# Siyou-Li/u2Tokenizer

Hardware: NVIDIA H100
Metric: ct_volumes_per_sec (higher is better)
Workload: dtype bf16

## Files before the change

include/u2b200.h:

```cpp
#ifndef U2B200_H_
#define U2B200_H_

#include <stdint.h>

#if defined(__GNUC__)
#define U2_API __attribute__((visibility("default")))
#else
#define U2_API
#endif

#ifdef __cplusplus
extern "C" {
#endif

#define U2_OK 0
#define U2_ERR_ARG (-1)
#define U2_ERR_CUDA (-2)
#define U2_ERR_UNSUPPORTED (-3)

#define U2_DT_BF16 0
#define U2_DT_F32 1

#define U2_ACT_NONE 0
#define U2_ACT_GELU 1
#define U2_ACT_SILU 2

#define U2_EPI_NONE 0
#define U2_EPI_EXP_ROW 1
#define U2_EPI_DS_ROW 2

U2_API int u2_version(void);
U2_API const char* u2_last_error(void);
U2_API int u2_device_sm_count(void);

typedef struct u2_gemm_desc {
  int32_t M, N, K;
  int32_t zi, zo;
  int32_t b_zi_div;
  int64_t lda, a_stride_zi, a_stride_zo;
  int64_t ldb, b_stride_zi, b_stride_zo;
  int64_t ldc, c_stride_zi, c_stride_zo;
  int32_t c_dtype;
  float alpha;
  const float* bias;
  int32_t act;
  const void* residual;
  int64_t ldr;
  int32_t res_row_mod;
  int32_t row_div, row_stride, row_off;
  int32_t block_n;
  int32_t a_mn, b_mn;
  int32_t epi_op;
  const float* rowvec;
  int64_t rv_stride_zi, rv_stride_zo;
  const void* mul;
} u2_gemm_desc;

U2_API int u2_gemm_bf16(const void* A, const void* B, void* C, const u2_gemm_desc* desc, void* stream);

U2_API int u2_layernorm_bf16(const void* x, const void* residual, const float* gamma, const float* beta,
                             void* y, void* sum_out, int64_t rows, int32_t E, int64_t ldx, int64_t ldr,
                             int64_t ldy, float eps, void* stream);
U2_API int u2_rmsnorm_bf16(const void* x, const void* residual, const float* gamma, void* y, void* sum_out,
                           int64_t rows, int32_t E, int64_t ldx, int64_t ldr, int64_t ldy, float eps,
                           void* stream);

// ... 271 lines not shown
```

u2tokenizer_b200/_lib.py:

```python
from __future__ import annotations

import ctypes as C
from pathlib import Path

_LIB_PATH = Path(__file__).resolve().parent / "libu2b200.so"
_lib = None


class GemmDesc(C.Structure):
    _fields_ = [
        ("M", C.c_int32), ("N", C.c_int32), ("K", C.c_int32),
        ("zi", C.c_int32), ("zo", C.c_int32), ("b_zi_div", C.c_int32),
        ("lda", C.c_int64), ("a_stride_zi", C.c_int64), ("a_stride_zo", C.c_int64),
        ("ldb", C.c_int64), ("b_stride_zi", C.c_int64), ("b_stride_zo", C.c_int64),
        ("ldc", C.c_int64), ("c_stride_zi", C.c_int64), ("c_stride_zo", C.c_int64),
        ("c_dtype", C.c_int32), ("alpha", C.c_float),
        ("bias", C.c_void_p),
        ("act", C.c_int32),
        ("residual", C.c_void_p),
        ("ldr", C.c_int64),
        ("res_row_mod", C.c_int32),
        ("row_div", C.c_int32), ("row_stride", C.c_int32), ("row_off", C.c_int32),
        ("block_n", C.c_int32),
        ("a_mn", C.c_int32), ("b_mn", C.c_int32),
# ... 176 lines not shown

BEAM_MAX_BEAMS, BEAM_MAX_EOS, BEAM_MAX_KEEP = 16, 8, 144


class BeamParams(C.Structure):
    _fields_ = [
        ("length_penalty", C.c_double),
        ("num_beams", C.c_int32), ("beams_to_keep", C.c_int32), ("early_stopping", C.c_int32),
        ("max_new_tokens", C.c_int32), ("n_eos", C.c_int32), ("reserved", C.c_int32),
        ("eos", C.c_int32 * BEAM_MAX_EOS),
    ]


class BeamStepDesc(C.Structure):
    _fields_ = [
        ("params", C.c_void_p),
        ("prompts", C.c_int32), ("V", C.c_int32),
        ("cand_val", C.c_void_p), ("cand_tok", C.c_void_p),
        ("running", C.c_void_p), ("fin_score", C.c_void_p), ("fin_info", C.c_void_p), ("flags", C.c_void_p),
        ("ids", C.c_void_p),
        ("rec", C.c_void_p), ("ld_rec", C.c_int64), ("rec_rows", C.c_int32),
        ("kv_src", C.c_void_p), ("ld_kv_src", C.c_int64),
        ("pos_dev", C.c_void_p),
        ("hist", C.c_void_p), ("ld_hist", C.c_int64), ("hist_cap", C.c_int32),
        ("step_dev", C.c_void_p),
    ]


_P, _I, _L, _F = C.c_void_p, C.c_int32, C.c_int64, C.c_float
SIGNATURES = {
    "u2_version": (C.c_int, []),
    "u2_last_error": (C.c_char_p, []),
    "u2_device_sm_count": (C.c_int, []),
    "u2_gemm_bf16": (C.c_int, [_P, _P, _P, C.POINTER(GemmDesc), _P]),
    "u2_layernorm_bf16": (C.c_int, [_P, _P, _P, _P, _P, _P, _L, _I, _L, _L, _L, _F, _P]),
    "u2_rmsnorm_bf16": (C.c_int, [_P, _P, _P, _P, _P, _L, _I, _L, _L, _L, _F, _P]),
    "u2_softmax_f32_bf16": (C.c_int, [_P, _P, C.POINTER(SoftmaxDesc), _P]),
    "u2_silu_mul_bf16": (C.c_int, [_P, _P, _L, _I, _L, _L, _I, _P]),
    "u2_patchify_f32_bf16": (C.c_int, [_P, _P, _L, _I, _I, _I, _I, _I, _I, _P]),
    "u2_patch_embed_f32_bf16": (C.c_int, [_P, _P, _P, _P, _P, _L, _I, _I, _I, _I, _I, _I, _I, _L, _P]),
    "u2_set_rows_bf16": (C.c_int, [_P, _P, _L, _L, _L, _I, _P]),
    "u2_vit_frame_rows_bf16": (C.c_int, [_P, _P, _L, _I, _I, _I, _P]),
    "u2_transpose_heads_bf16": (C.c_int, [_P, _P, _I, _I, _I, _I, _L, _L, _L, _L, _L, _L, _P]),
    "u2_spp_pool_bf16": (C.c_int, [_P, _P, _L, _I, _I, _I, _I, _I, _L, _L, _L, _I, _P]),
    "u2_multiscale_pool_bf16": (C.c_int, [_P, _P, _P, _F, _P, _I, _I, _I, _I, _P]),
    "u2_multiscale_pool_ws_elems": (C.c_int64, [_I, _I]),
    "u2_embed_splice_bf16": (C.c_int, [_P, _P, _P, _P, _I, _I, _I, _I, _L, _P]),
    "u2_temporal_attention_bf16": (C.c_int, [_P, _P, _I, _I, _I, _I, _I, _L, _L, _F, _P, _I, _P]),
    "u2_rope_bf16": (C.c_int, [_P, C.POINTER(RopeDesc), _P]),
    "u2_decode_attention_bf16": (C.c_int, [_P, _P, _P, _P, _I, _I, _I, _I, _I, _I, _P, _L, _L, _F, _I, _P, _L, _P]),
    "u2_decode_attention_window_bf16": (C.c_int, [_P, _P, _P, _P, _I, _I, _I, _I, _I, _I, _P, _L, _L, _F, _I, _P, _L,
                                                  _I, _P]),
    "u2_gemv_bf16": (C.c_int, [_P, _P, _P, C.POINTER(GemvDesc), _P]),
    "u2_argmax_f32": (C.c_int, [_P, _P, _P, _I, _I, _L, _P]),
    "u2_dlinear_bf16": (C.c_int, [_P, _P, _P, C.POINTER(DlinearDesc), _P]),
    "u2_decode_attention_fused_bf16": (C.c_int, [_P, _P, _P, _P, C.POINTER(FusedDecodeDesc), _P]),
    "u2_decode_embed_bf16": (C.c_int, [_P, _P, _P, _P, _P, _P, _P, _P, _I, _I, _L, _P]),
    "u2_flash_attention_d64_bf16": (C.c_int, [_P, _P, _P, _P, C.POINTER(FaDesc), _P]),
    "u2_sample_f32": (C.c_int, [_P, _P, _I, _I, _L, _F, _I, _F, C.c_uint64, _P, _I, _P]),
    "u2_sample_dev_f32": (C.c_int, [_P, _P, _I, _I, _L, _P, _P, _I, _P]),
    "u2_logits_process_f32": (C.c_int, [_P, _I, _I, _L, _P, _P, _L, _I, _P, _P, _I, _P]),
    "u2_topk_rows_f32": (C.c_int, [_P, _P, _I, _I, _I, _L, _L, _P]),
    "u2_log_softmax_f32": (C.c_int, [_P, _P, _I, _I, _L, _L, _P]),
    "u2_beam_topk_f32": (C.c_int, [_P, _L, _I, _I, _P, _P, _P, _P, _P, _P]),
    "u2_beam_step": (C.c_int, [C.POINTER(BeamStepDesc), _I, _P]),
    "u2_dlinear_ws_elems": (C.c_int64, [_I, _I]),
# ... 79 lines not shown
```

u2tokenizer_b200/csrc/attn_small.cu:

```cuda
#include <cooperative_groups.h>
#include <cuda_bf16.h>
#include <math.h>

#include <type_traits>

#include "host_util.h"
#include "u2b200.h"

namespace u2 {

__device__ __forceinline__ float wsum(float v) {
#pragma unroll
  for (int o = 16; o > 0; o >>= 1) v += __shfl_xor_sync(0xffffffffu, v, o);
  return v;
}
__device__ __forceinline__ float wmax(float v) {
#pragma unroll
  for (int o = 16; o > 0; o >>= 1) v = fmaxf(v, __shfl_xor_sync(0xffffffffu, v, o));
  return v;
}

__global__ void __launch_bounds__(128)
temporal_attention_kernel(const __nv_bfloat16* __restrict__ qkv, __nv_bfloat16* __restrict__ out, int C, int N,
                          int H, int dh, long long ld_qkv, long long ld_out, float scale,
// ... 545 lines not shown
      }
    }
  }
#pragma unroll
  for (int g = 0; g < kG; ++g) {
    if (lane == 0) {
      s_m[warp][g] = m[g];
      s_l[warp][g] = l[g];
    }
    if (kLanes == 32 || lane < kLanes) {
#pragma unroll
      for (int i = 0; i < kEpl; ++i) s_acc[warp][g][lane * kEpl + i] = acc[g][i];
    }
  }
  __syncthreads();
  for (int idx = threadIdx.x; idx < kG * kDh; idx += blockDim.x) {
    const int g = idx / kDh, e = idx - g * kDh;
    float gm = -INFINITY;
#pragma unroll
    for (int w = 0; w < kFaWarps; ++w) gm = fmaxf(gm, s_m[w][g]);
    float gl = 0.f, o = 0.f;
#pragma unroll
    for (int w = 0; w < kFaWarps; ++w) {
      if (s_m[w][g] != -INFINITY) {
        const float f = __expf(s_m[w][g] - gm);
        gl += s_l[w][g] * f;
        o += s_acc[w][g][e] * f;
      }
    }
    a.out[(long long)b * a.ldo + (long long)(hk * kG + g) * kDh + e] = __float2bfloat16(o / gl);
  }
}

template <int kDh, int kG, bool kInd, bool kWin = false>
__global__ void __launch_bounds__(256)
fused_decode_attention_split_kernel(const FusedArgsT<kInd, kWin> a) {
  namespace cg = cooperative_groups;
  cg::cluster_group cluster = cg::this_cluster();
  constexpr int kW = 8;
  constexpr int kEpl = PvMap<kDh>::kEpl;
  constexpr int kLanes = PvMap<kDh>::kLanes;
  constexpr int kVw = (kEpl + 1) / 2;
  const int S = (int)gridDim.z, rank = (int)blockIdx.z;
  const int hk = blockIdx.x, b = blockIdx.y;
  const int warp = threadIdx.x >> 5, lane = threadIdx.x & 31;
  const int le = kLanes == 32 ? lane : min(lane, kLanes - 1);
  asm volatile("griddepcontrol.launch_dependents;" ::: "memory");
  const int pos = a.pos_dev ? a.pos_dev[a.pos_per_seq ? b : 0] : a.pos_host;
  const int T = min(pos + 1, a.Tmax);
  const int lo = window_lo<kWin>(a, pos);
  __shared__ __align__(16) float s_q[kG][kDh];
  __shared__ __align__(16) __nv_bfloat16 s_knew[kDh];
  __shared__ __align__(16) __nv_bfloat16 s_vnew[kDh];
  __shared__ float s_m[kW][kG], s_l[kW][kG];
  __shared__ float s_acc[kW][kG][kDh];
  __shared__ float c_m[kG], c_l[kG];
  __shared__ __align__(16) float c_o[kG][kDh];

  const __nv_bfloat16* row = a.qkv + (long long)b * a.ldq;
  __nv_bfloat16* kbase = a.kc + ((long long)b * a.Hkv + hk) * a.Tmax * kDh;
  __nv_bfloat16* vbase = a.vc + ((long long)b * a.Hkv + hk) * a.Tmax * kDh;

  uint4 ku[kDh / 8];
  uint32_t vw[32][kVw];
  int t0 = (lo & ~31) + (warp * S + rank) * 32;
  const long long row_elems = (long long)a.Hkv * a.Tmax * kDh;
  auto request = [&](int base) {
    const int t = min(base + lane, T - 1);
    const long long dsrc = kv_src_delta<kInd>(a, b, t, pos, row_elems);
    const uint4* kr = reinterpret_cast<const uint4*>(kbase + (long long)t * kDh + dsrc);
#pragma unroll
    for (int c = 0; c < kDh / 8; ++c) ku[c] = kr[c];
#pragma unroll
    for (int jj = 0; jj < 32; ++jj) {
      const int tj = min(base + jj, T - 1);
      long long dj = 0;
      if constexpr (kInd) dj = __shfl_sync(0xffffffffu, dsrc, tj - base);
      const __nv_bfloat16* vp = vbase + (long long)tj * kDh + dj + le * kEpl;
      if constexpr (kEpl == 4) {
        const uint2 u = *reinterpret_cast<const uint2*>(vp);
        vw[jj][0] = u.x;
        vw[jj][1] = u.y;
      } else if constexpr (kEpl == 2) {
        vw[jj][0] = *reinterpret_cast<const uint32_t*>(vp);
      } else {
        vw[jj][0] = *reinterpret_cast<const unsigned short*>(vp);
      }
    }
  };
  if (t0 < T) request(t0);
  asm volatile("griddepcontrol.wait;" ::: "memory");

  for (int job = warp; job < kG + 2; job += kW) {
    if (job == kG) {
      norm_rope_head<kDh>(row + (long long)(a.Hq + hk) * kDh, a.k_norm_w, a.eps, a.inv_freq, pos, 1.f, nullptr, s_knew, lane);
      __syncwarp();
      if (rank == 0)
        for (int e = lane; e < kDh; e += 32) kbase[(long long)pos * kDh + e] = s_knew[e];
    } else if (job == kG + 1) {
      const __nv_bfloat16* v = row + (long long)(a.Hq + a.Hkv + hk) * kDh;
      for (int e = lane; e < kDh; e += 32) {
        const __nv_bfloat16 x = v[e];
        s_vnew[e] = x;
        if (rank == 0) vbase[(long long)pos * kDh + e] = x;
      }
    } else {
      norm_rope_head<kDh>(row + (long long)(hk * kG + job) * kDh, a.q_norm_w, a.eps, a.inv_freq, pos, a.scale, s_q[job],
                          nullptr, lane);
    }
  }
  __syncthreads();

  float m[kG], l[kG], acc[kG][kEpl];
#pragma unroll
  for (int g = 0; g < kG; ++g) {
    m[g] = -INFINITY;
    l[g] = 0.f;
#pragma unroll
    for (int i = 0; i < kEpl; ++i) acc[g][i] = 0.f;
  }
  while (t0 < T) {
    const int t = t0 + lane;
    if (t == pos) {
#pragma unroll
      for (int c = 0; c < kDh / 8; ++c) ku[c] = reinterpret_cast<const uint4*>(s_knew)[c];
    }
    float s[kG];
#pragma unroll
    for (int g = 0; g < kG; ++g) s[g] = 0.f;
#pragma unroll
    for (int c = 0; c < kDh / 8; ++c) {
      const __nv_bfloat162* h2 = reinterpret_cast<const __nv_bfloat162*>(&ku[c]);
      float kf[8];
#pragma unroll
      for (int j = 0; j < 4; ++j) {
        const float2 f2 = __bfloat1622float2(h2[j]);
        kf[2 * j] = f2.x;
        kf[2 * j + 1] = f2.y;
      }
#pragma unroll
      for (int g = 0; g < kG; ++g) {
        const float4 q0 = *reinterpret_cast<const float4*>(&s_q[g][c * 8]);
        const float4 q1 = *reinterpret_cast<const float4*>(&s_q[g][c * 8 + 4]);
        s[g] += kf[0] * q0.x + kf[1] * q0.y + kf[2] * q0.z + kf[3] * q0.w + kf[4] * q1.x + kf[5] * q1.y + kf[6] * q1.z +
                kf[7] * q1.w;
      }
    }
    float p[kG];
    const bool vis = t < T && (!kWin || t >= lo);
#pragma unroll
    for (int g = 0; g < kG; ++g) {
      if (!vis) s[g] = -INFINITY;
      const float mx = fmaxf(m[g], wmax(s[g]));
      const float corr = __expf(m[g] - mx);
      p[g] = vis ? __expf(s[g] - mx) : 0.f;
      l[g] = l[g] * corr + wsum(p[g]);
#pragma unroll
      for (int i = 0; i < kEpl; ++i) acc[g][i] *= corr;
      m[g] = mx;
    }
#pragma unroll
    for (int jj = 0; jj < 32; ++jj) {
      float vf[kEpl];
      if (t0 + jj == pos) {
#pragma unroll
        for (int i = 0; i < kEpl; ++i) vf[i] = __bfloat162float(s_vnew[le * kEpl + i]);
      } else if constexpr (kEpl == 4) {
        const float2 x = __bfloat1622float2(*reinterpret_cast<const __nv_bfloat162*>(&vw[jj][0]));
        const float2 y = __bfloat1622float2(*reinterpret_cast<const __nv_bfloat162*>(&vw[jj][1]));
        vf[0] = x.x; vf[1] = x.y; vf[2] = y.x; vf[3] = y.y;
      } else if constexpr (kEpl == 2) {
        const float2 x = __bfloat1622float2(*reinterpret_cast<const __nv_bfloat162*>(&vw[jj][0]));
        vf[0] = x.x; vf[1] = x.y;
      } else {
        vf[0] = __uint_as_float(vw[jj][0] << 16);
      }
#pragma unroll
      for (int g = 0; g < kG; ++g) {
        const float pj = __shfl_sync(0xffffffffu, p[g], jj);
#pragma unroll
        for (int i = 0; i < kEpl; ++i) acc[g][i] += pj * vf[i];
      }
    }
    t0 += S * kW * 32;
    if (t0 < T) request(t0);
  }
#pragma unroll
  for (int g = 0; g < kG; ++g) {
    if (lane == 0) {
      s_m[warp][g] = m[g];
      s_l[warp][g] = l[g];
    }
    if (kLanes == 32 || lane < kLanes) {
#pragma unroll
      for (int i = 0; i < kEpl; ++i) s_acc[warp][g][lane * kEpl + i] = acc[g][i];
    }
  }
  __syncthreads();
  for (int idx = threadIdx.x; idx < kG * kDh; idx += blockDim.x) {
    const int g = idx / kDh, e = idx - g * kDh;
    float gm = -INFINITY;
#pragma unroll
    for (int w = 0; w < kW; ++w) gm = fmaxf(gm, s_m[w][g]);
    float gl = 0.f, o = 0.f;
#pragma unroll
    for (int w = 0; w < kW; ++w) {
      if (s_m[w][g] != -INFINITY) {
        const float f = __expf(s_m[w][g] - gm);
        gl += s_l[w][g] * f;
        o += s_acc[w][g][e] * f;
      }
    }
    c_o[g][e] = o;
    if (e == 0) {
      c_m[g] = gm;
      c_l[g] = gl;
    }
  }
  cluster.sync();
  if (rank == 0) {
    for (int idx = threadIdx.x; idx < kG * kDh; idx += blockDim.x) {
      const int g = idx / kDh, e = idx - g * kDh;
      float gm = -INFINITY;
      for (int r = 0; r < S; ++r) gm = fmaxf(gm, *cluster.map_shared_rank(&c_m[g], r));
      float gl = 0.f, o = 0.f;
      for (int r = 0; r < S; ++r) {
        const float mr = *cluster.map_shared_rank(&c_m[g], r);
        if (mr != -INFINITY) {
          const float f = __expf(mr - gm);
          gl += *cluster.map_shared_rank(&c_l[g], r) * f;
          o += *cluster.map_shared_rank(&c_o[g][e], r) * f;
        }
      }
      a.out[(long long)b * a.ldo + (long long)(hk * kG + g) * kDh + e] = __float2bfloat16(o / gl);
    }
  }
  cluster.sync();
}

template <int kDh, int kG, bool kInd, bool kWin>
static int launch_fused_decode_split(const FusedArgsT<kInd, kWin>& a, dim3 grid, bool pdl, cudaStream_t st) {
  cudaLaunchConfig_t cfg = {};
  cfg.gridDim = grid;
  cfg.blockDim = dim3(256);
  cfg.dynamicSmemBytes = 0;
  cfg.stream = st;
  cudaLaunchAttribute attr[2];
  attr[0].id = cudaLaunchAttributeClusterDimension;
  attr[0].val.clusterDim.x = 1;
  attr[0].val.clusterDim.y = 1;
  attr[0].val.clusterDim.z = grid.z;
  attr[1].id = cudaLaunchAttributeProgrammaticStreamSerialization;
  attr[1].val.programmaticStreamSerializationAllowed = 1;
  cfg.attrs = attr;
  cfg.numAttrs = pdl ? 2 : 1;
  cudaError_t e = cudaLaunchKernelEx(&cfg, fused_decode_attention_split_kernel<kDh, kG, kInd, kWin>, a);
  if (e != cudaSuccess) return set_error(U2_ERR_CUDA, "decode_attention_fused (split-KV) launch: %s", cudaGetErrorString(e));
  return U2_OK;
}

template <int kDh, bool kInd, bool kWin = false>
static int launch_fused_decode(const FusedArgsT<kInd, kWin>& a, int G, dim3 grid, bool pdl, cudaStream_t st) {
  if (grid.z > 1) {
    switch (G) {
      case 1: return launch_fused_decode_split<kDh, 1, kInd, kWin>(a, grid, pdl, st);
      case 2: return launch_fused_decode_split<kDh, 2, kInd, kWin>(a, grid, pdl, st);
      case 4: return launch_fused_decode_split<kDh, 4, kInd, kWin>(a, grid, pdl, st);
      case 8: return launch_fused_decode_split<kDh, 8, kInd, kWin>(a, grid, pdl, st);
      default: return set_error(U2_ERR_UNSUPPORTED, "decode_attention_fused: Hq/Hkv = %d (supported 1, 2, 4, 8)", G);
    }
  }
  switch (G) {
    case 1: fused_decode_attention_kernel<kDh, 1, kInd, kWin><<<grid, FaCfg<kDh, 1>::kWarps * 32, 0, st>>>(a); break;
    case 2: fused_decode_attention_kernel<kDh, 2, kInd, kWin><<<grid, FaCfg<kDh, 2>::kWarps * 32, 0, st>>>(a); break;
    case 4: fused_decode_attention_kernel<kDh, 4, kInd, kWin><<<grid, FaCfg<kDh, 4>::kWarps * 32, 0, st>>>(a); break;
    case 8: fused_decode_attention_kernel<kDh, 8, kInd, kWin><<<grid, FaCfg<kDh, 8>::kWarps * 32, 0, st>>>(a); break;
    default: return set_error(U2_ERR_UNSUPPORTED, "decode_attention_fused: Hq/Hkv = %d (supported 1, 2, 4, 8)", G);
  }
  return U2_OK;
}

template <int kDh>
static int launch_fused_decode(const FusedDecodeWinArgs& a, int G, dim3 grid, bool pdl, cudaStream_t st) {
  if (a.window > 0) {
    if (a.kv_src) return launch_fused_decode<kDh, true, true>(a, G, grid, pdl, st);
    return launch_fused_decode<kDh, false, true>(a, G, grid, pdl, st);
  }
  if (a.kv_src) return launch_fused_decode<kDh, true>(static_cast<const FusedDecodeIndArgs&>(a), G, grid, pdl, st);
  return launch_fused_decode<kDh, false>(static_cast<const FusedDecodeArgs&>(a), G, grid, pdl, st);
// ... 42 lines not shown
```

u2tokenizer_b200/csrc/dlinear_wgmma.cu:

```cuda
#include <cuda_bf16.h>
#include <math.h>
#include <stdio.h>
#include <stdlib.h>

#include "host_util.h"
#include "ptx.cuh"
#include "u2b200.h"

namespace u2 {

constexpr int kDlN = 16;
constexpr int kDlK = 64;
constexpr int kDlBBytes = kDlN * kDlK * 2;
constexpr int kDlThreads = 384;
constexpr int kDlMmaWarp0 = 8;
constexpr int kDlAccLd = 20;

template <int kM>
struct DlCfg {
  static constexpr int kABytes = kM * kDlK * 2;
  static constexpr int kStageBytes = kABytes + kDlBBytes;
#ifndef U2_DL_STAGES128
#define U2_DL_STAGES128 10
#endif
  static constexpr int kStages = (kM == 128) ? U2_DL_STAGES128 : 18;
  static constexpr int kAccBytes = 2 * kM * kDlAccLd * 4;
  static constexpr int kSmem = kStages * kStageBytes + kAccBytes + 1024 + 512;
};

struct DlinArgs {
  int B, N, K;
  int num_tiles, kblocks;
  float* ws;
  int max_slots;
  int* counters;
  const float* ssq_in;
  float inv_norm_dim, eps;
  const __nv_bfloat16* residual;
  long long ldr;
  void* y;
  long long ldy;
  int y_dtype;
  int silu_pair;
  const float* gamma_next;
  __nv_bfloat16* xg;
  long long ldxg;
  float* ssq_out;
  float* ssq_part;
  int* ssq_ticket;
// ... 92 lines not shown
      it.kb = 0;
      it.left = 0;
    } else {
      const long long base = units * blockIdx.x / G;
      const long long end = units * (blockIdx.x + 1) / G;
      it.tile = (int)(base / kblocks);
      it.kb = (int)(base - (long long)it.tile * kblocks);
      it.left = (int)(end - base);
    }
  }
  return it;
}

__device__ __forceinline__ void wait_tile_flag(const int* flags, int t, int step, unsigned char* ready, int tag) {
  if (ready[t] == (unsigned char)tag) return;
  const int t4 = t & ~3;
  for (;;) {
    int4 f;
    asm volatile("ld.relaxed.gpu.global.v4.s32 {%0, %1, %2, %3}, [%4];"
                 : "=r"(f.x), "=r"(f.y), "=r"(f.z), "=r"(f.w)
                 : "l"(flags + t4)
                 : "memory");
    if (f.x >= step) ready[t4] = (unsigned char)tag;
    if (f.y >= step) ready[t4 + 1] = (unsigned char)tag;
    if (f.z >= step) ready[t4 + 2] = (unsigned char)tag;
    if (f.w >= step) ready[t4 + 3] = (unsigned char)tag;
    if (ready[t] == (unsigned char)tag) break;
  }
  asm volatile("fence.acq_rel.gpu;" ::: "memory");
  asm volatile("fence.proxy.async;" ::: "memory");
}

template <int kM>
__global__ void __launch_bounds__(kDlThreads, 1)
dlinear_wgmma_kernel(const __grid_constant__ DlinMulti mp) {
  using Cfg = DlCfg<kM>;
  constexpr int kStages = Cfg::kStages;
  constexpr int kABytes = Cfg::kABytes;
  constexpr int kStageBytes = Cfg::kStageBytes;
  constexpr bool kTiles = (kM == 64);
  extern __shared__ uint8_t smem_raw[];
  uint8_t* smem = reinterpret_cast<uint8_t*>((reinterpret_cast<uintptr_t>(smem_raw) + 1023) & ~static_cast<uintptr_t>(1023));
  uint8_t* smem_a = smem;
  uint8_t* smem_b = smem + kStages * kABytes;
  float* smem_acc = reinterpret_cast<float*>(smem + kStages * kStageBytes);
  uint64_t* bars = reinterpret_cast<uint64_t*>(smem + kStages * kStageBytes + Cfg::kAccBytes);
  uint64_t* full_bar = bars;
  uint64_t* empty_bar = bars + kStages;
  uint64_t* acc_full_bar = bars + 2 * kStages;
  uint64_t* acc_empty_bar = bars + 2 * kStages + 2;
  __shared__ unsigned char s_ready[1024];
  if (threadIdx.x < 256) reinterpret_cast<unsigned int*>(s_ready)[threadIdx.x] = 0u;

  const int warp_idx = threadIdx.x / 32;
  const int lane = threadIdx.x % 32;
  const int n_ops = mp.n_ops;

  if (warp_idx == 0 && lane == 0) {
    for (int i = 0; i < n_ops; ++i) {
      tma_prefetch_desc(&mp.tw[i]);
      tma_prefetch_desc(&mp.tx[i]);
    }
  }
  if (warp_idx == 1 && lane == 0) {
    for (int s = 0; s < kStages; ++s) {
      mbar_init(&full_bar[s], 1);
      mbar_init(&empty_bar[s], 4);
// ... 145 lines not shown
    uint32_t acc_phase = 0;
    for (int oi = 0; oi < n_ops; ++oi) {
      const DlinArgs& p = mp.op[oi];
      UnitIter it = make_iter(p.num_tiles, p.kblocks, kTiles);
      bool prev_done = (oi == 0);
      if (oi > 0 && !p.dep_flags) {
        if (et == 0) grid_barrier_wait(mp.gridbar + (oi - 1), target);
        asm volatile("bar.sync 1, 128;" ::: "memory");
        prev_done = true;
      }
      while (it.left > 0) {
        const int tile = it.tile;
        const int seg_kb = it.seg_len();
        it.left -= seg_kb;
        it.kb += seg_kb;
        if (it.kb == it.kblocks) {
          it.kb = 0;
          it.tile += it.tile_step;
        }

        const int row = tile * kM + trow;
        const bool whole = (seg_kb == p.kblocks);
        int gf = (int)blockIdx.x, n_contrib = 0;
        if (!whole) {
          const long long units = (long long)p.num_tiles * p.kblocks;
          const long long G = units < (long long)gridDim.x ? units : (long long)gridDim.x;
          const long long u0 = (long long)tile * p.kblocks;
          gf = (int)(((u0 + 1) * G + units - 1) / units) - 1;
          n_contrib = (int)(((u0 + p.kblocks) * G + units - 1) / units) - 1 - gf;
        }
        const bool finalizer = (gf == (int)blockIdx.x);
        const int nvec = (p.B + 3) >> 2;
        const bool row_ok = tvalid && row < p.N;
        unsigned short res_raw[16];
        float rs[16];
        float gam = 0.f;
        if (finalizer) {
          if (!prev_done) {
            if (et == 0) grid_barrier_wait(mp.gridbar + (oi - 1), target);
            asm volatile("bar.sync 1, 128;" ::: "memory");
            prev_done = true;
          }
#pragma unroll
          for (int b = 0; b < 16; ++b) {
            res_raw[b] = 0;
            rs[b] = 1.f;
            if (b < p.B) {
              if (p.residual && !p.silu_pair && row_ok)
                res_raw[b] = __ldcg(reinterpret_cast<const unsigned short*>(p.residual) + (long long)b * p.ldr + row);
              if (p.ssq_in) rs[b] = __ldcg(p.ssq_in + b);
            }
          }
          if (p.gamma_next && row_ok) gam = __ldg(p.gamma_next + row);
        }

        mbar_wait(&acc_full_bar[acc], acc_phase);
        if (et == 0 && it.left == 0) U2_STAMP(oi, 4);
        uint32_t v[16];
        {
          const uint32_t src = smem_u32(smem_acc + acc * (kM * kDlAccLd) + trow * kDlAccLd);
#pragma unroll
          for (int c = 0; c < 4; ++c) {
            const uint4 x = lds128(src + 16 * c);
            v[4 * c] = x.x; v[4 * c + 1] = x.y; v[4 * c + 2] = x.z; v[4 * c + 3] = x.w;
          }
        }
        __syncwarp();
        if ((threadIdx.x & 31) == 0) mbar_arrive(&acc_empty_bar[acc]);
        if (++acc == 2) {
          acc = 0;
          acc_phase ^= 1;
        }

        float f[16];
#pragma unroll
        for (int b = 0; b < 16; ++b) f[b] = __uint_as_float(v[b]);
        if (!finalizer) {
          const int slot = (int)blockIdx.x - gf - 1;
          float4* dst = reinterpret_cast<float4*>(p.ws + (((long long)tile * p.max_slots + slot) * kM + trow) * kDlN);
          if (tvalid) {
#pragma unroll
            for (int c = 0; c < 4; ++c)
              if (c < nvec) __stcg(dst + c, make_float4(f[4 * c], f[4 * c + 1], f[4 * c + 2], f[4 * c + 3]));
          }
        } else {
// ... 4 lines not shown
            const float4 sent = make_float4(__uint_as_float(0xffffffffu), __uint_as_float(0xffffffffu),
                                            __uint_as_float(0xffffffffu), __uint_as_float(0xffffffffu));
#pragma unroll
            for (int c = 0; c < 4; ++c) {
              if (c >= nvec) break;
              constexpr int kMaxSlots = 8;
              for (int s0 = 0; s0 < n_contrib; s0 += kMaxSlots) {
                float4 t[kMaxSlots];
                bool ok;
                unsigned int spins = 0;
                do {
                  ok = true;
#pragma unroll
                  for (int sl = 0; sl < kMaxSlots; ++sl)
                    if (s0 + sl < n_contrib) t[sl] = ld_relaxed_f4(src0 + (s0 + sl) * slot_stride + c);
#pragma unroll
                  for (int sl = 0; sl < kMaxSlots; ++sl)
                    if (s0 + sl < n_contrib) {
                      ok = ok && (__float_as_uint(t[sl].x) != 0xffffffffu) && (__float_as_uint(t[sl].y) != 0xffffffffu) &&
                           (__float_as_uint(t[sl].z) != 0xffffffffu) && (__float_as_uint(t[sl].w) != 0xffffffffu);
                    }
                } while (!ok && ++spins < (1u << 22));
#pragma unroll
                for (int sl = 0; sl < kMaxSlots; ++sl)
                  if (s0 + sl < n_contrib) {
                    f[4 * c] += t[sl].x; f[4 * c + 1] += t[sl].y; f[4 * c + 2] += t[sl].z; f[4 * c + 3] += t[sl].w;
                    __stcg(src0 + (s0 + sl) * slot_stride + c, sent);
                  }
              }
            }
          }
          if (et == 0) U2_STAMP(oi, 7);
          if (p.ssq_zero && tile == 0 && et < 16) p.ssq_zero[et] = 0.f;
          float sq[16];
#pragma unroll
          for (int b = 0; b < 16; ++b) {
            sq[b] = 0.f;
            if (b < p.B) {
              float val = f[b];
              if (p.ssq_in) val *= rsqrtf(rs[b] * p.inv_norm_dim + p.eps);
              if (p.silu_pair) {
                const float me = __bfloat162float(__float2bfloat16(val));
                const float other = __shfl_down_sync(0xffffffffu, me, 1);
                if (row_ok && (trow & 1) == 0) {
                  const float o = __fdividef(me, 1.f + __expf(-me)) * other;
                  reinterpret_cast<__nv_bfloat16*>(p.y)[(long long)b * p.ldy + (row >> 1)] = __float2bfloat16(o);
                }
              } else if (row_ok) {
                val += __bfloat162float(__ushort_as_bfloat16(res_raw[b]));
                if (p.y_dtype == U2_DT_BF16) {
                  const __nv_bfloat16 o = __float2bfloat16(val);
                  reinterpret_cast<__nv_bfloat16*>(p.y)[(long long)b * p.ldy + row] = o;
                  val = __bfloat162float(o);
                } else {
                  reinterpret_cast<float*>(p.y)[(long long)b * p.ldy + row] = val;
                }
                if (p.gamma_next) p.xg[(long long)b * p.ldxg + row] = __float2bfloat16(val * gam);
                sq[b] = val * val;
              }
            }
          }
          if (p.ssq_out) {
            __shared__ float s_sq[4][16];
            __shared__ int s_last;
#pragma unroll
            for (int b = 0; b < 16; ++b) {
              float s = sq[b];
#pragma unroll
              for (int o = 16; o > 0; o >>= 1) s += __shfl_xor_sync(0xffffffffu, s, o);
              if (lane == 0) s_sq[q][b] = s;
            }
            asm volatile("bar.sync 1, 128;" ::: "memory");
            if (et < 16) {
              __stcg(p.ssq_part + (long long)tile * 16 + et, ((s_sq[0][et] + s_sq[1][et]) + s_sq[2][et]) + s_sq[3][et]);
              __threadfence();
            }
            asm volatile("bar.sync 1, 128;" ::: "memory");
            if (et == 0) s_last = (atomicAdd(p.ssq_ticket, 1) == p.num_tiles - 1);
            asm volatile("bar.sync 1, 128;" ::: "memory");
            if (s_last) {
              __shared__ float s_grp[8][16];
              __threadfence();
              const int col = et & 15, grp = et >> 4;
              float t = 0.f;
              for (int i0 = grp; i0 < p.num_tiles; i0 += 32) {
                float v[4];
#pragma unroll
                for (int u = 0; u < 4; ++u) {
                  const int i = i0 + 8 * u;
                  v[u] = (i < p.num_tiles) ? __ldcg(p.ssq_part + (long long)i * 16 + col) : 0.f;
                }
#pragma unroll
                for (int u = 0; u < 4; ++u) {
                  const int i = i0 + 8 * u;
                  if (i < p.num_tiles) {
                    t += v[u];
                    __stcg(p.ssq_part + (long long)i * 16 + col, __uint_as_float(0xffffffffu));
                  }
                }
              }
              s_grp[grp][col] = t;
              asm volatile("bar.sync 1, 128;" ::: "memory");
              if (et < p.B) {
                float tot = 0.f;
// ... 118 lines not shown
static int launch_multi_t(DlinMulti& mp, int pdl, cudaStream_t stream) {
  static bool configured = false;
  if (!configured) {
    cudaError_t e = cudaFuncSetAttribute(dlinear_wgmma_kernel<kM>, cudaFuncAttributeMaxDynamicSharedMemorySize, DlCfg<kM>::kSmem);
    if (e != cudaSuccess) return set_error(U2_ERR_CUDA, "dlinear: cudaFuncSetAttribute: %s", cudaGetErrorString(e));
    int per_sm = 0;
    e = cudaOccupancyMaxActiveBlocksPerMultiprocessor(&per_sm, dlinear_wgmma_kernel<kM>, kDlThreads, DlCfg<kM>::kSmem);
    if (e != cudaSuccess || per_sm < 1)
      return set_error(U2_ERR_CUDA, "dlinear: kernel cannot be resident on an SM (%s, %d CTA/SM): set U2_MULTI_OP=0",
                       cudaGetErrorString(e), per_sm);
    configured = true;
  }
  int grid = num_sms();
  if (grid <= 0) return set_error(U2_ERR_CUDA, "dlinear: cannot query SM count");
  if (mp.n_ops == 1) {
    const long long work = (kM == 64) ? mp.op[0].num_tiles : (long long)mp.op[0].num_tiles * mp.op[0].kblocks;
    if (work < grid) grid = (int)work;
  }
  cudaLaunchConfig_t cfg = {};
  cfg.gridDim = dim3((unsigned)grid);
  cfg.blockDim = dim3(kDlThreads);
  cfg.dynamicSmemBytes = DlCfg<kM>::kSmem;
  cfg.stream = stream;
  cudaLaunchAttribute attr[1];
  attr[0].id = cudaLaunchAttributeProgrammaticStreamSerialization;
  attr[0].val.programmaticStreamSerializationAllowed = 1;
  cfg.attrs = attr;
  cfg.numAttrs = pdl ? 1 : 0;
  cudaError_t e = cudaLaunchKernelEx(&cfg, dlinear_wgmma_kernel<kM>, mp);
  if (e != cudaSuccess) return set_error(U2_ERR_CUDA, "dlinear launch: %s", cudaGetErrorString(e));
  return U2_OK;
}

static int launch_multi(DlinMulti& mp, int kM, int pdl, cudaStream_t stream) {
  return kM == 64 ? launch_multi_t<64>(mp, pdl, stream) : launch_multi_t<128>(mp, pdl, stream);
}

static inline int tile_m_of(const u2_dlinear_desc* d) { return d->sched == U2_DLIN_TILES64 ? 64 : 128; }


extern "C" U2_API int64_t u2_dlinear_ws_elems(int32_t N, int32_t K) {
  if (N <= 0 || K <= 0) return 0;
  const long long tiles = (N + 127) / 128, kblocks = (K + kDlK - 1) / kDlK;
  int g = num_sms();
  if (g <= 0) g = 132;
  long long rmin = tiles * kblocks / g;
  if (rmin < 1) rmin = 1;
  const long long cmax = (kblocks + rmin - 1) / rmin + 1;
  return tiles * cmax * 128 * kDlN + (N + 63) / 64 * kDlN;
}

extern "C" U2_API int u2_dlinear_bf16(const void* x, const void* w, void* y, const u2_dlinear_desc* d, void* stream) {
  static DlinMulti mp;
  mp.n_ops = 1;
  if (!d) return set_error(U2_ERR_ARG, "dlinear: null descriptor");
  const int kM = tile_m_of(d);
  int rc = fill_op(x, w, y, d, &mp.op[0], &mp.tw[0], &mp.tx[0], kM);
  if (rc) return rc;
  mp.gridbar = nullptr;
  mp.n_next = 0;
  mp.lookahead_units = 0;
  mp.pre_stages = 0;
  mp.dbg = reinterpret_cast<unsigned long long*>(d->dbg);
  mp.step_dev = d->counters;
  return launch_multi(mp, kM, d->pdl, reinterpret_cast<cudaStream_t>(stream));
}
// ... 48 lines not shown
```

u2tokenizer_b200/csrc/host_util.cu:

```cuda
#include "host_util.h"

#include <stdarg.h>
#include <stdio.h>
#include <string.h>

#include "u2b200.h"

namespace u2 {

static thread_local char g_err[512] = "";

int set_error(int code, const char* fmt, ...) {
  va_list ap;
  va_start(ap, fmt);
  vsnprintf(g_err, sizeof(g_err), fmt, ap);
  va_end(ap);
  return code;
}

const char* last_error() { return g_err; }

int num_sms() {
  static int cached[64] = {0};
  int dev = 0;
// ... 90 lines not shown
  cuuint64_t strides[2] = {(cuuint64_t)(stride1_elems * 4), (cuuint64_t)(stride2_elems * 4)};
  cuuint32_t box[3] = {(cuuint32_t)box0, (cuuint32_t)box1, (cuuint32_t)box2};
  cuuint32_t estr[3] = {1, 1, 1};
  CUresult r = enc(out, CU_TENSOR_MAP_DATA_TYPE_FLOAT32, 3, const_cast<void*>(base), dims, strides,
                   box, estr, CU_TENSOR_MAP_INTERLEAVE_NONE, CU_TENSOR_MAP_SWIZZLE_NONE,
                   CU_TENSOR_MAP_L2_PROMOTION_L2_256B, CU_TENSOR_MAP_FLOAT_OOB_FILL_NONE);
  if (r != CUDA_SUCCESS) return set_error(U2_ERR_CUDA, "cuTensorMapEncodeTiled(f32 3d) failed: %d", (int)r);
  return U2_OK;
}

int make_tmap_f32_nd(CUtensorMap* out, const void* base, int n, const int64_t* dims, const int64_t* strides_bytes,
                     const int* box) {
  EncodeTiledFn enc = get_encode();
  if (!enc) return set_error(U2_ERR_CUDA, "cuTensorMapEncodeTiled entry point not available");
  if (n < 1 || n > 5) return set_error(U2_ERR_ARG, "tensor map rank %d", n);
  cuuint64_t d[5], st[4];
  cuuint32_t bx[5], es[5];
  for (int i = 0; i < n; ++i) { d[i] = (cuuint64_t)dims[i]; bx[i] = (cuuint32_t)box[i]; es[i] = 1; }
  for (int i = 0; i + 1 < n; ++i) st[i] = (cuuint64_t)strides_bytes[i];
  CUresult r = enc(out, CU_TENSOR_MAP_DATA_TYPE_FLOAT32, (cuuint32_t)n, const_cast<void*>(base), d, st, bx, es,
                   CU_TENSOR_MAP_INTERLEAVE_NONE, CU_TENSOR_MAP_SWIZZLE_NONE, CU_TENSOR_MAP_L2_PROMOTION_L2_256B,
                   CU_TENSOR_MAP_FLOAT_OOB_FILL_NONE);
  if (r != CUDA_SUCCESS) return set_error(U2_ERR_CUDA, "cuTensorMapEncodeTiled(f32 %d-d) failed: %d", n, (int)r);
  return U2_OK;
}

}

namespace u2 { const char* last_error(); }

extern "C" U2_API int u2_version(void) { return 1; }
extern "C" U2_API const char* u2_last_error(void) { return u2::last_error(); }
extern "C" U2_API int u2_device_sm_count(void) { return u2::num_sms(); }
```

u2tokenizer_b200/csrc/host_util.h:

```cpp
#pragma once
#include <cuda.h>
#include <cuda_runtime.h>
#include <stdint.h>

namespace u2 {

int set_error(int code, const char* fmt, ...);
int num_sms();

int make_tmap_bf16_4d(CUtensorMap* out, const void* base, int64_t k, int64_t rows, int64_t zi,
                      int64_t zo, int64_t ld, int64_t stride_zi, int64_t stride_zo, int box_k,
                      int box_rows);

int make_tmap_store_4d(CUtensorMap* out, void* base, int elem_bytes, int64_t n, int64_t rows, int64_t zi, int64_t zo,
                       int64_t ld, int64_t stride_zi, int64_t stride_zo, int box_n, int box_rows);

int make_tmap_f32_3d(CUtensorMap* out, const void* base, int64_t d0, int64_t d1, int64_t d2,
                     int64_t stride1_elems, int64_t stride2_elems, int box0, int box1, int box2);

int make_tmap_f32_nd(CUtensorMap* out, const void* base, int n, const int64_t* dims, const int64_t* strides_bytes,
                     const int* box);

}

#define U2_CHECK_LAUNCH(what)                                                          \
  do {                                                                                 \
    cudaError_t e__ = cudaGetLastError();                                              \
    if (e__ != cudaSuccess)                                                            \
      return ::u2::set_error(U2_ERR_CUDA, "%s: %s", what, cudaGetErrorString(e__));   \
  } while (0)
```

u2tokenizer_b200/engine.py:

```python
from __future__ import annotations

import math
from dataclasses import asdict, dataclass, replace
from typing import Dict, List, Optional, Tuple

import torch

from . import _lib, ops
from .geometry import Geometry

BF16, F32 = torch.bfloat16, torch.float32
REL_MAX = 512


def _pad8(n: int) -> int:
    return (n + 7) // 8 * 8


@dataclass(frozen=True)
class LogitsProcessors:
    repetition_penalty: float = 1.0
    no_repeat_ngram_size: int = 0
    min_new_tokens: int = 0
    eos_token_ids: Tuple[int, ...] = ()
# ... 72 lines not shown
    wqkv: torch.Tensor
    bqkv: torch.Tensor
    wd: torch.Tensor
    bd: torch.Tensor
    rel: Optional[torch.Tensor]
    seq_first: bool = False


@dataclass
class _CrossAttnW:
    wq: torch.Tensor
    bq: torch.Tensor
    wkv: torch.Tensor
    bkv: torch.Tensor
    wd: Optional[torch.Tensor]
    bd: Optional[torch.Tensor]


class U2Engine:
    def __init__(self, geom: Geometry, state_dict: Dict[str, torch.Tensor], device="cuda",
                 attn_workspace_bytes: int = 6 << 30, decode_impl: str = "tcgen05"):
        if not torch.cuda.is_available():
            raise RuntimeError("U2Engine needs a CUDA device: the hot path has no CPU implementation")
        from . import _lib
        _lib.load()
        self.g = geom
        self.dev = torch.device(device)
        self.attn_ws = attn_workspace_bytes
        self.decode_impl = decode_impl
        import os
        from . import _lib
        self.num_sms = int(_lib.load().u2_device_sm_count())
        self.fwd_graph = os.environ.get("U2_FWD_GRAPH", "1") != "0"
        self.attn_pdl = os.environ.get("U2_ATTN_PDL", "0") != "0"
        self.pdl = os.environ.get("U2_PDL", "1") != "0"
        self.multi_op = os.environ.get("U2_MULTI_OP", "1") != "0"
        self.fused_patch_embed = os.environ.get("U2_FUSED_PATCH_EMBED", "0") != "0"
        self.use_flash = os.environ.get("U2_FLASH", "1") != "0"
        self.fine_deps = os.environ.get("U2_FINE_DEPS", "0") != "0"
        self.dl_sched = int(os.environ.get("U2_DL_SCHED", "0"))
        self.pre_stages = int(os.environ.get("U2_PRE_STAGES", "0"))
        self.l2_lookahead_units = int(os.environ.get("U2_L2_LOOKAHEAD", "0"))
        self.l2_next_units = int(os.environ.get("U2_L2_NEXT", "-1"))
        if geom.vision_select_feature != "patch":
            raise NotImplementedError("only vision_select_feature='patch' is supported (the spp projector needs it)")
        t = _Take(dict(state_dict), self.dev)
        self._prep_vit(t)
        self._prep_projector(t)
        if geom.enable_u2tokenizer:
            self._prep_tokenizer(t)
        self._prep_decoder(t)
        self._gen_state = None
        self._fwd_state = None
        self._param_blocks = {}
        self.last_beam_scores = None

    def _prep_vit(self, t: _Take):
        g = self.g
        v = "model.vision_tower.vision_tower."
        self.pe_w = t.bf(v + "patch_embedding.patch_embeddings.1.weight")
        self.pe_b = t.f32(v + "patch_embedding.patch_embeddings.1.bias")
        self.pos = t.bf(v + "patch_embedding.position_embeddings").view(g.n_patches, g.vit_hidden)
        self.cls = t.bf(v + "cls_token").view(g.vit_hidden)
        self.vit = []
        for i in range(g.vit_layers):
            b = f"{v}blocks.{i}."
            self.vit.append(dict(
# ... 450 lines not shown
        pairs = B * self.g.num_key_value_heads
        s = 8
        while s > 1 and pairs * s > max(self.num_sms, pairs):
            s //= 2
        return s

    def _use_tc_decode(self, B: int) -> bool:
        g = self.g
        dims = (g.hidden_size, g.intermediate_size, g.num_attention_heads * g.head_dim)
        return self.decode_impl == "tcgen05" and B <= 16 and all(k % 64 == 0 for k in dims)

    def _decode_rows(self) -> int:
        tc_rows = 16
        return tc_rows if self._use_tc_decode(tc_rows) else 8

    def decode_step_tc(self, cache: "KVCache", req: Optional[GenerateRequest] = None) -> torch.Tensor:
        g = self.g
        B = cache.batch
        hq, hkv, dh = g.num_attention_heads, g.num_key_value_heads, g.head_dim
        bufs = self._decode_buffers(B)
        x, qkv, ctx, act, logits, ids, xg_a, xg_b = (bufs[k] for k in ("x", "qkv", "ctx", "act", "logits", "ids", "xg", "xg2"))
        ssq_a, ssq_b, ws, cnt, flags = bufs["ssq_a"], bufs["ssq_b"], bufs["ws"], bufs["counters"], bufs["flags"]
        gridbar, step = bufs["gridbar"], bufs["step"]
        eps = g.rms_norm_eps
        nl = len(self.layers)
        c0 = dict(ws=ws[0], counters=cnt[0], sched=self.dl_sched)
        c1 = dict(ws=ws[1], counters=cnt[1], sched=self.dl_sched)
        ops.decode_embed(ids, self.embed, self.layers[0]["ln1"], x, xg_b, ssq_b, ssq_a, step)
        ops.dlinear(xg_b, self.layers[0]["wqkv"], qkv, ssq_in=ssq_b, eps=eps, pdl=self.pdl, **c1)
        for li, w in enumerate(self.layers):
            ops.decode_attention_fused(qkv, cache.k[li], cache.v[li], ctx, B=B, Hq=hq, Hkv=hkv, dh=dh, Tmax=cache.max_len,
                                       inv_freq=self.inv_freq, scale=1.0 / math.sqrt(dh), pos_dev=cache.length_dev,
                                       q_norm_w=w["qn"], k_norm_w=w["kn"], eps=eps, kv_splits=self._kv_splits(B),
                                       pdl=self.pdl and self.attn_pdl, pos_per_seq=True, kv_src=cache.kv_src,
                                       window=g.window)
            last = li + 1 == nl
            g_next = self.final_norm if last else self.layers[li + 1]["ln1"]
            fl = flags[li] if (self.multi_op and self.fine_deps) else [None] * 4
            dep = lambda i, shift: dict(dep_flags=fl[i], dep_shift=shift) if fl[i] is not None else {}
            chain = [
                (ctx, w["wo"], x, dict(residual=x, gamma_next=w["ln2"], xg=xg_a, ssq_out=ssq_a, ssq_zero=ssq_b,
                                       out_flags=fl[0], **c0)),
                (xg_a, w["wgu"], act, dict(ssq_in=ssq_a, eps=eps, silu_pair=True, out_flags=fl[1], **dep(0, 1), **c1)),
                (act, w["wdown"], x, dict(residual=x, gamma_next=g_next, xg=xg_b, ssq_out=ssq_b, ssq_zero=ssq_a,
                                          out_flags=fl[2], **dep(1, 0), **c0)),
                (xg_b, self.lm_head, logits, dict(ssq_in=ssq_b, eps=eps, **dep(2, 1), **c1)) if last else
                (xg_b, self.layers[li + 1]["wqkv"], qkv, dict(ssq_in=ssq_b, eps=eps, **dep(2, 1), **c1)),
            ]
            if self.multi_op:
                nxt = () if (last or self.l2_next_units < 0) else (
                    (self.layers[li + 1]["wo"], 1 << 20), (self.layers[li + 1]["wgu"], self.l2_next_units))
                ops.dlinear_multi(chain, gridbar=gridbar[li * 4:(li + 1) * 4], step_dev=step, pdl=self.pdl,
                                  lookahead_units=self.l2_lookahead_units, next_weights=nxt,
                                  pre_stages=self.pre_stages)
            else:
                for (xi, wi, yi, kw) in chain:
                    ops.dlinear(xi, wi, yi, pdl=self.pdl, **kw)
        self._pick_next(logits, ids.view(B), bufs["step"], req)
        cache.advance_device()
        return logits

    def _pick_next(self, logits: torch.Tensor, ids_out: torch.Tensor, step_dev: Optional[torch.Tensor],
                   req: Optional[GenerateRequest], step: int = 0):
        if req is not None and req.beam is not None:
            return self._beam_pick(logits, ids_out, step_dev, req, step)
        if req is not None and req.processors is not None:
            blk = self._param_block("logits processors", ops.logits_proc_params, self.g.vocab_size,
# ... 295 lines not shown
```

Before: 2.166.

## Co-schedule decode attention beside dlinear chain with register-capped small variant

```diff
diff --git a/include/u2b200.h b/include/u2b200.h
--- a/include/u2b200.h
+++ b/include/u2b200.h
@@ -32,6 +32,9 @@
 U2_API int u2_version(void);
 U2_API const char* u2_last_error(void);
 U2_API int u2_device_sm_count(void);
+U2_API int32_t u2_coresident_fits(int32_t regs_a, int32_t threads_a, int32_t smem_a, int32_t regs_b, int32_t threads_b,
+                                  int32_t smem_b, int32_t sm_regs, int32_t sm_smem, int32_t sm_threads,
+                                  int32_t smem_reserved);
 
 typedef struct u2_gemm_desc {
   int32_t M, N, K;
diff --git a/u2tokenizer_b200/_lib.py b/u2tokenizer_b200/_lib.py
--- a/u2tokenizer_b200/_lib.py
+++ b/u2tokenizer_b200/_lib.py
@@ -232,6 +232,7 @@
     "u2_version": (C.c_int, []),
     "u2_last_error": (C.c_char_p, []),
     "u2_device_sm_count": (C.c_int, []),
+    "u2_coresident_fits": (C.c_int32, [_I] * 10),
     "u2_gemm_bf16": (C.c_int, [_P, _P, _P, C.POINTER(GemmDesc), _P]),
     "u2_layernorm_bf16": (C.c_int, [_P, _P, _P, _P, _P, _P, _L, _I, _L, _L, _L, _F, _P]),
     "u2_rmsnorm_bf16": (C.c_int, [_P, _P, _P, _P, _P, _L, _I, _L, _L, _L, _F, _P]),
diff --git a/u2tokenizer_b200/csrc/attn_small.cu b/u2tokenizer_b200/csrc/attn_small.cu
--- a/u2tokenizer_b200/csrc/attn_small.cu
+++ b/u2tokenizer_b200/csrc/attn_small.cu
@@ -601,9 +601,9 @@
   }
 }
 
-template <int kDh, int kG, bool kInd, bool kWin = false>
-__global__ void __launch_bounds__(256)
-fused_decode_attention_split_kernel(const FusedArgsT<kInd, kWin> a) {
+constexpr int kFaSmallRegs = 152;
+template <int kDh, int kG, bool kInd, bool kWin, int kPW>
+__device__ __forceinline__ void fused_decode_attention_split_body(const FusedArgsT<kInd, kWin>& a) {
   namespace cg = cooperative_groups;
   cg::cluster_group cluster = cg::this_cluster();
   constexpr int kW = 8;
@@ -634,14 +634,10 @@
   uint32_t vw[32][kVw];
   int t0 = (lo & ~31) + (warp * S + rank) * 32;
   const long long row_elems = (long long)a.Hkv * a.Tmax * kDh;
-  auto request = [&](int base) {
-    const int t = min(base + lane, T - 1);
-    const long long dsrc = kv_src_delta<kInd>(a, b, t, pos, row_elems);
-    const uint4* kr = reinterpret_cast<const uint4*>(kbase + (long long)t * kDh + dsrc);
-#pragma unroll
-    for (int c = 0; c < kDh / 8; ++c) ku[c] = kr[c];
-#pragma unroll
-    for (int jj = 0; jj < 32; ++jj) {
+  constexpr int kVpre = kPW == 8 ? 32 : 16;
+  auto request_v = [&](int base, int jlo, int jhi, long long dsrc) {
+#pragma unroll
+    for (int jj = jlo; jj < jhi; ++jj) {
       const int tj = min(base + jj, T - 1);
       long long dj = 0;
       if constexpr (kInd) dj = __shfl_sync(0xffffffffu, dsrc, tj - base);
@@ -657,10 +653,18 @@
       }
     }
   };
+  auto request = [&](int base) {
+    const int t = min(base + lane, T - 1);
+    const long long dsrc = kv_src_delta<kInd>(a, b, t, pos, row_elems);
+    const uint4* kr = reinterpret_cast<const uint4*>(kbase + (long long)t * kDh + dsrc);
+#pragma unroll
+    for (int c = 0; c < kDh / 8; ++c) ku[c] = kr[c];
+    request_v(base, 0, kVpre, dsrc);
+  };
   if (t0 < T) request(t0);
   asm volatile("griddepcontrol.wait;" ::: "memory");
 
-  for (int job = warp; job < kG + 2; job += kW) {
+  for (int job = warp; job < kG + 2; job += kPW) {
     if (job == kG) {
       norm_rope_head<kDh>(row + (long long)(a.Hq + hk) * kDh, a.k_norm_w, a.eps, a.inv_freq, pos, 1.f, nullptr, s_knew, lane);
       __syncwarp();
@@ -680,6 +684,11 @@
   }
   __syncthreads();
 
+  for (int pw = warp; pw < kW; pw += kPW) {
+  if (pw != warp) {
+    t0 = (lo & ~31) + (pw * S + rank) * 32;
+    if (t0 < T) request(t0);
+  }
   float m[kG], l[kG], acc[kG][kEpl];
 #pragma unroll
   for (int g = 0; g < kG; ++g) {
@@ -715,6 +724,7 @@
                 kf[7] * q1.w;
       }
     }
+    if constexpr (kVpre < 32) request_v(t0, kVpre, 32, kv_src_delta<kInd>(a, b, min(t, T - 1), pos, row_elems));
     float p[kG];
     const bool vis = t < T && (!kWin || t >= lo);
 #pragma unroll
@@ -757,13 +767,14 @@
 #pragma unroll
   for (int g = 0; g < kG; ++g) {
     if (lane == 0) {
-      s_m[warp][g] = m[g];
-      s_l[warp][g] = l[g];
+      s_m[pw][g] = m[g];
+      s_l[pw][g] = l[g];
     }
     if (kLanes == 32 || lane < kLanes) {
 #pragma unroll
-      for (int i = 0; i < kEpl; ++i) s_acc[warp][g][lane * kEpl + i] = acc[g][i];
-    }
+      for (int i = 0; i < kEpl; ++i) s_acc[pw][g][lane * kEpl + i] = acc[g][i];
+    }
+  }
   }
   __syncthreads();
   for (int idx = threadIdx.x; idx < kG * kDh; idx += blockDim.x) {
@@ -807,11 +818,27 @@
   cluster.sync();
 }
 
+template <int kDh, int kG, bool kInd, bool kWin = false>
+__global__ void __launch_bounds__(256)
+fused_decode_attention_split_kernel(const FusedArgsT<kInd, kWin> a) {
+  fused_decode_attention_split_body<kDh, kG, kInd, kWin, 8>(a);
+}
+
+template <int kDh, int kG, bool kInd, bool kWin = false>
+__global__ void __maxnreg__(kFaSmallRegs)
+fused_decode_attention_split4_kernel(const FusedArgsT<kInd, kWin> a) {
+  fused_decode_attention_split_body<kDh, kG, kInd, kWin, 4>(a);
+}
+
 template <int kDh, int kG, bool kInd, bool kWin>
 static int launch_fused_decode_split(const FusedArgsT<kInd, kWin>& a, dim3 grid, bool pdl, cudaStream_t st) {
+  static int small_fits = -1;
+  if (pdl && small_fits < 0)
+    small_fits = fits_beside_decode_chain(reinterpret_cast<const void*>(fused_decode_attention_split4_kernel<kDh, kG, kInd, kWin>), 128);
+  const bool small = pdl && small_fits == 1;
   cudaLaunchConfig_t cfg = {};
   cfg.gridDim = grid;
-  cfg.blockDim = dim3(256);
+  cfg.blockDim = dim3(small ? 128 : 256);
   cfg.dynamicSmemBytes = 0;
   cfg.stream = st;
   cudaLaunchAttribute attr[2];
@@ -822,8 +849,9 @@
   attr[1].id = cudaLaunchAttributeProgrammaticStreamSerialization;
   attr[1].val.programmaticStreamSerializationAllowed = 1;
   cfg.attrs = attr;
-  cfg.numAttrs = pdl ? 2 : 1;
-  cudaError_t e = cudaLaunchKernelEx(&cfg, fused_decode_attention_split_kernel<kDh, kG, kInd, kWin>, a);
+  cfg.numAttrs = small ? 2 : 1;
+  cudaError_t e = small ? cudaLaunchKernelEx(&cfg, fused_decode_attention_split4_kernel<kDh, kG, kInd, kWin>, a)
+                        : cudaLaunchKernelEx(&cfg, fused_decode_attention_split_kernel<kDh, kG, kInd, kWin>, a);
   if (e != cudaSuccess) return set_error(U2_ERR_CUDA, "decode_attention_fused (split-KV) launch: %s", cudaGetErrorString(e));
   return U2_OK;
 }
diff --git a/u2tokenizer_b200/csrc/dlinear_wgmma.cu b/u2tokenizer_b200/csrc/dlinear_wgmma.cu
--- a/u2tokenizer_b200/csrc/dlinear_wgmma.cu
+++ b/u2tokenizer_b200/csrc/dlinear_wgmma.cu
@@ -15,6 +15,7 @@
 constexpr int kDlThreads = 384;
 constexpr int kDlMmaWarp0 = 8;
 constexpr int kDlAccLd = 20;
+constexpr int kDlMaxRegs = 120;
 
 template <int kM>
 struct DlCfg {
@@ -173,7 +174,7 @@
 }
 
 template <int kM>
-__global__ void __launch_bounds__(kDlThreads, 1)
+__global__ void __maxnreg__(kDlMaxRegs)
 dlinear_wgmma_kernel(const __grid_constant__ DlinMulti mp) {
   using Cfg = DlCfg<kM>;
   constexpr int kStages = Cfg::kStages;
@@ -385,8 +386,8 @@
         const bool finalizer = (gf == (int)blockIdx.x);
         const int nvec = (p.B + 3) >> 2;
         const bool row_ok = tvalid && row < p.N;
-        unsigned short res_raw[16];
-        float rs[16];
+        uint32_t res2[8];
+        float rs_lane = 1.f;
         float gam = 0.f;
         if (finalizer) {
           if (!prev_done) {
@@ -395,15 +396,16 @@
             prev_done = true;
           }
 #pragma unroll
-          for (int b = 0; b < 16; ++b) {
-            res_raw[b] = 0;
-            rs[b] = 1.f;
-            if (b < p.B) {
-              if (p.residual && !p.silu_pair && row_ok)
-                res_raw[b] = __ldcg(reinterpret_cast<const unsigned short*>(p.residual) + (long long)b * p.ldr + row);
-              if (p.ssq_in) rs[b] = __ldcg(p.ssq_in + b);
+          for (int b2 = 0; b2 < 8; ++b2) {
+            uint32_t lo = 0, hi = 0;
+            if (p.residual && !p.silu_pair && row_ok) {
+              const unsigned short* r = reinterpret_cast<const unsigned short*>(p.residual) + row;
+              if (2 * b2 < p.B) lo = __ldcg(r + (long long)(2 * b2) * p.ldr);
+              if (2 * b2 + 1 < p.B) hi = __ldcg(r + (long long)(2 * b2 + 1) * p.ldr);
             }
-          }
+            res2[b2] = lo | (hi << 16);
+          }
+          if (p.ssq_in && lane < p.B) rs_lane = __ldcg(p.ssq_in + lane);
           if (p.gamma_next && row_ok) gam = __ldg(p.gamma_next + row);
         }
 
@@ -474,13 +476,13 @@
           }
           if (et == 0) U2_STAMP(oi, 7);
           if (p.ssq_zero && tile == 0 && et < 16) p.ssq_zero[et] = 0.f;
-          float sq[16];
+          __shared__ float s_sq[4][16];
 #pragma unroll
           for (int b = 0; b < 16; ++b) {
-            sq[b] = 0.f;
+            float sq = 0.f;
             if (b < p.B) {
               float val = f[b];
-              if (p.ssq_in) val *= rsqrtf(rs[b] * p.inv_norm_dim + p.eps);
+              if (p.ssq_in) val *= rsqrtf(__shfl_sync(0xffffffffu, rs_lane, b) * p.inv_norm_dim + p.eps);
               if (p.silu_pair) {
                 const float me = __bfloat162float(__float2bfloat16(val));
                 const float other = __shfl_down_sync(0xffffffffu, me, 1);
@@ -489,7 +491,7 @@
                   reinterpret_cast<__nv_bfloat16*>(p.y)[(long long)b * p.ldy + (row >> 1)] = __float2bfloat16(o);
                 }
               } else if (row_ok) {
-                val += __bfloat162float(__ushort_as_bfloat16(res_raw[b]));
+                val += __bfloat162float(__ushort_as_bfloat16((unsigned short)(res2[b >> 1] >> (16 * (b & 1)))));
                 if (p.y_dtype == U2_DT_BF16) {
                   const __nv_bfloat16 o = __float2bfloat16(val);
                   reinterpret_cast<__nv_bfloat16*>(p.y)[(long long)b * p.ldy + row] = o;
@@ -498,20 +500,19 @@
                   reinterpret_cast<float*>(p.y)[(long long)b * p.ldy + row] = val;
                 }
                 if (p.gamma_next) p.xg[(long long)b * p.ldxg + row] = __float2bfloat16(val * gam);
-                sq[b] = val * val;
+                sq = val * val;
               }
             }
+            if (p.ssq_out) {
+              if (b < p.B) {
+#pragma unroll
+                for (int o = 16; o > 0; o >>= 1) sq += __shfl_xor_sync(0xffffffffu, sq, o);
+              }
+              if (lane == 0) s_sq[q][b] = sq;
+            }
           }
           if (p.ssq_out) {
-            __shared__ float s_sq[4][16];
             __shared__ int s_last;
-#pragma unroll
-            for (int b = 0; b < 16; ++b) {
-              float s = sq[b];
-#pragma unroll
-              for (int o = 16; o > 0; o >>= 1) s += __shfl_xor_sync(0xffffffffu, s, o);
-              if (lane == 0) s_sq[q][b] = s;
-            }
             asm volatile("bar.sync 1, 128;" ::: "memory");
             if (et < 16) {
               __stcg(p.ssq_part + (long long)tile * 16 + et, ((s_sq[0][et] + s_sq[1][et]) + s_sq[2][et]) + s_sq[3][et]);
@@ -696,6 +697,34 @@
   return U2_OK;
 }
 
+namespace u2 {
+int fits_beside_decode_chain(const void* kernel, int threads) {
+  int dev = 0, sm_regs = 0, sm_smem = 0, sm_threads = 0, reserved = 0;
+  if (cudaGetDevice(&dev) != cudaSuccess ||
+      cudaDeviceGetAttribute(&sm_regs, cudaDevAttrMaxRegistersPerMultiprocessor, dev) != cudaSuccess ||
+      cudaDeviceGetAttribute(&sm_smem, cudaDevAttrMaxSharedMemoryPerMultiprocessor, dev) != cudaSuccess ||
+      cudaDeviceGetAttribute(&sm_threads, cudaDevAttrMaxThreadsPerMultiProcessor, dev) != cudaSuccess ||
+      cudaDeviceGetAttribute(&reserved, cudaDevAttrReservedSharedMemoryPerBlock, dev) != cudaSuccess)
+    return 0;
+  cudaFuncAttributes fa;
+  int per_sm = 0;
+  if (cudaFuncGetAttributes(&fa, kernel) != cudaSuccess ||
+      cudaOccupancyMaxActiveBlocksPerMultiprocessor(&per_sm, kernel, threads, 0) != cudaSuccess || per_sm < 1)
+    return 0;
+  const void* chains[2] = {reinterpret_cast<const void*>(dlinear_wgmma_kernel<128>),
+                           reinterpret_cast<const void*>(dlinear_wgmma_kernel<64>)};
+  const int chain_dyn[2] = {DlCfg<128>::kSmem, DlCfg<64>::kSmem};
+  for (int i = 0; i < 2; ++i) {
+    cudaFuncAttributes ca;
+    if (cudaFuncGetAttributes(&ca, chains[i]) != cudaSuccess) return 0;
+    if (!u2_coresident_fits(ca.numRegs, kDlThreads, (int)ca.sharedSizeBytes + chain_dyn[i], fa.numRegs, threads,
+                            (int)fa.sharedSizeBytes, sm_regs, sm_smem, sm_threads, reserved))
+      return 0;
+  }
+  return 1;
+}
+}
+
 static int launch_multi(DlinMulti& mp, int kM, int pdl, cudaStream_t stream) {
   return kM == 64 ? launch_multi_t<64>(mp, pdl, stream) : launch_multi_t<128>(mp, pdl, stream);
 }
diff --git a/u2tokenizer_b200/csrc/host_util.cu b/u2tokenizer_b200/csrc/host_util.cu
--- a/u2tokenizer_b200/csrc/host_util.cu
+++ b/u2tokenizer_b200/csrc/host_util.cu
@@ -146,3 +146,14 @@
 extern "C" U2_API int u2_version(void) { return 1; }
 extern "C" U2_API const char* u2_last_error(void) { return u2::last_error(); }
 extern "C" U2_API int u2_device_sm_count(void) { return u2::num_sms(); }
+
+extern "C" U2_API int32_t u2_coresident_fits(int32_t regs_a, int32_t threads_a, int32_t smem_a, int32_t regs_b,
+                                             int32_t threads_b, int32_t smem_b, int32_t sm_regs, int32_t sm_smem,
+                                             int32_t sm_threads, int32_t smem_reserved) {
+  if (regs_a <= 0 || regs_b <= 0 || threads_a <= 0 || threads_b <= 0 || smem_a < 0 || smem_b < 0) return 0;
+  if (threads_a + threads_b > sm_threads) return 0;
+  if ((long long)smem_a + smem_b + 2LL * smem_reserved > sm_smem) return 0;
+  const long long warp_a = ((long long)regs_a * 32 + 255) / 256 * 256, warp_b = ((long long)regs_b * 32 + 255) / 256 * 256;
+  const long long quad = warp_a * ((threads_a + 127) / 128) + warp_b * ((threads_b + 127) / 128);
+  return quad <= sm_regs / 4 ? 1 : 0;
+}
diff --git a/u2tokenizer_b200/csrc/host_util.h b/u2tokenizer_b200/csrc/host_util.h
--- a/u2tokenizer_b200/csrc/host_util.h
+++ b/u2tokenizer_b200/csrc/host_util.h
@@ -7,6 +7,7 @@
 
 int set_error(int code, const char* fmt, ...);
 int num_sms();
+int fits_beside_decode_chain(const void* kernel, int threads);
 
 int make_tmap_bf16_4d(CUtensorMap* out, const void* base, int64_t k, int64_t rows, int64_t zi,
                       int64_t zo, int64_t ld, int64_t stride_zi, int64_t stride_zo, int box_k,
diff --git a/u2tokenizer_b200/engine.py b/u2tokenizer_b200/engine.py
--- a/u2tokenizer_b200/engine.py
+++ b/u2tokenizer_b200/engine.py
@@ -128,7 +128,6 @@
         from . import _lib
         self.num_sms = int(_lib.load().u2_device_sm_count())
         self.fwd_graph = os.environ.get("U2_FWD_GRAPH", "1") != "0"
-        self.attn_pdl = os.environ.get("U2_ATTN_PDL", "0") != "0"
         self.pdl = os.environ.get("U2_PDL", "1") != "0"
         self.multi_op = os.environ.get("U2_MULTI_OP", "1") != "0"
         self.fused_patch_embed = os.environ.get("U2_FUSED_PATCH_EMBED", "0") != "0"
@@ -645,7 +644,7 @@
             ops.decode_attention_fused(qkv, cache.k[li], cache.v[li], ctx, B=B, Hq=hq, Hkv=hkv, dh=dh, Tmax=cache.max_len,
                                        inv_freq=self.inv_freq, scale=1.0 / math.sqrt(dh), pos_dev=cache.length_dev,
                                        q_norm_w=w["qn"], k_norm_w=w["kn"], eps=eps, kv_splits=self._kv_splits(B),
-                                       pdl=self.pdl and self.attn_pdl, pos_per_seq=True, kv_src=cache.kv_src,
+                                       pdl=self.pdl and self.multi_op, pos_per_seq=True, kv_src=cache.kv_src,
                                        window=g.window)
             last = li + 1 == nl
             g_next = self.final_norm if last else self.layers[li + 1]["ln1"]
```

Result: no change. 2.171 (median of 6 runs) (+0.2%).
